# atomicarchitects/equiformer

Measured on NVIDIA H100. Metric: edges/sec fwd+bwd, QM9 Lmax=2 batch, higher is better.
Workload: dtype f32

## Files before the change

### equiformer_b200/csrc/eqf_gemm_tf32x3.cu

```cuda
#include <cuda.h>
#include <cuda_runtime.h>

#include <cstdint>
#include <cstdlib>
#include <mutex>
#include <string>

#include "eqf_common.cuh"
#include "eqf_tc.cuh"

namespace eqf {
namespace tf32x3 {

using namespace tc;

constexpr int BM = 128;
constexpr int BK = kKTile;
constexpr int kRowBytes = BK * 4;
constexpr int kThreads = 384;
constexpr int kConsumerWarps = 8, kConsumerThreads = kConsumerWarps * 32;
constexpr int kSmemBudget = 227 * 1024;
constexpr int kMaxStages = 8;

template <int BN>
// ... 48 lines not shown
    if (++kt == k_tiles) { kt = 0; tile += gridDim.x; }
    const bool more = tile < n_tiles;
    if (more) {
      mbar_wait_hint(&full[s], ph);
      load_a_split(smem_u32(smem + s * S::kStageBytes), row_wg, lane, hn, ln);
    }
    wgmma_wait<0>();
    __syncwarp();
    if (lane == 0) mbar_arrive(&empty[s_cur]);
#pragma unroll
    for (int i = 0; i < BN / 2; ++i) acc[i] = kt_cur == 0 ? part[i] : acc[i] + part[i];
    if (kt_cur == k_tiles - 1) {
      if (leader) bulk_wait_read();
      named_barrier(wg, 128);
      stage_acc<BN>(acc, out, row_w, lane);
      fence_async_smem();
      named_barrier(wg, 128);
      if (leader) {
        const int m0 = (int)(tile_cur / n_blocks) * BM + (wg - 1) * 64;
        const int n0 = (int)(tile_cur % n_blocks) * BN;
#pragma unroll
        for (int b = 0; b < BN / 32; ++b) tma_store_2d(map_c, n0 + 32 * b, m0, out + (uint32_t)b * 8192u);
        bulk_commit();
      }
    }
    return more;
  }
};

template <int BN>
__global__ void __launch_bounds__(kThreads, 1)
gemm_tf32x3_kernel(const __grid_constant__ CUtensorMap map_a, const __grid_constant__ CUtensorMap map_bhi,
                   const __grid_constant__ CUtensorMap map_blo, const __grid_constant__ CUtensorMap map_c, Params p) {
  using S = Smem<BN>;
  constexpr int kStages = S::kStages;
  extern __shared__ uint8_t smem_raw[];
  uint8_t* smem = reinterpret_cast<uint8_t*>((reinterpret_cast<uintptr_t>(smem_raw) + 1023) & ~uintptr_t(1023));
  uint8_t* out_base = smem + kStages * S::kStageBytes;
  uint64_t* full = reinterpret_cast<uint64_t*>(out_base + 2 * S::kOutBytes);
  uint64_t* empty = full + kStages;

  const int warp = threadIdx.x >> 5, lane = threadIdx.x & 31, wg = warp >> 2;
  const int k_tiles = (p.K + BK - 1) / BK;
  if (threadIdx.x == 0) {
    for (int s = 0; s < kStages; ++s) { mbar_init(&full[s], 1); mbar_init(&empty[s], kConsumerWarps); }
    asm volatile("fence.mbarrier_init.release.cluster;" ::: "memory");
  }
  __syncthreads();

  if (wg == 0) {
    reg_dealloc<40>();
    if (threadIdx.x == 0) {
      prefetch_map(&map_a); prefetch_map(&map_bhi); prefetch_map(&map_blo);
      int s = 0;
      uint32_t ph = 0;
      for (long long tile = blockIdx.x; tile < p.n_tiles; tile += gridDim.x) {
        const int m0 = (int)(tile / p.n_blocks) * BM;
        const int n0 = (int)(tile % p.n_blocks) * BN;
        for (int kt = 0; kt < k_tiles; ++kt) {
          mbar_wait_hint(&empty[s], ph ^ 1);
          uint8_t* st = smem + s * S::kStageBytes;
          mbar_expect_tx(&full[s], (uint32_t)S::kStageBytes);
          tma_load_2d(st, &map_a, kt * BK, m0, &full[s]);
          tma_load_2d(st + S::kABytes, &map_bhi, kt * BK, n0, &full[s]);
          tma_load_2d(st + S::kABytes + S::kBBytes, &map_blo, kt * BK, n0, &full[s]);
          if (++s == kStages) { s = 0; ph ^= 1; }
        }
      }
    }
  } else {
    reg_alloc<232>();
    if ((long long)blockIdx.x >= p.n_tiles) return;
    Consumer<BN> c;
    c.smem = smem; c.full = full; c.empty = empty; c.map_c = &map_c;
    c.out = smem_u32(out_base + (wg - 1) * S::kOutBytes);
    c.tile = blockIdx.x; c.n_tiles = p.n_tiles; c.kt = 0; c.k_tiles = k_tiles; c.n_blocks = p.n_blocks;
    c.s = 0; c.ph = 0; c.lane = lane; c.wg = wg;
    c.row_w = (warp & 3) * 16;
    c.row_wg = (wg - 1) * 64 + c.row_w;
    c.leader = (threadIdx.x & 127) == 0;
    if (c.leader) prefetch_map(&map_c);
    uint32_t h0[16], l0[16], h1[16], l1[16];
    mbar_wait_hint(&full[0], 0);
    load_a_split(smem_u32(smem), c.row_wg, lane, h0, l0);
    while (c.step(h0, l0, h1, l1) && c.step(h1, l1, h0, l0)) {}
    if (c.leader) bulk_wait();
  }
}

__global__ void split_kernel(const float* __restrict__ w, float* __restrict__ hi, float* __restrict__ lo, long long n) {
  for (long long i = (long long)blockIdx.x * blockDim.x + threadIdx.x; i < n; i += (long long)gridDim.x * blockDim.x) {
    const float v = w[i];
    const float h = tf32_rn(v);
    hi[i] = h;
    lo[i] = tf32_rn(v - h);
  }
}

__global__ void split_transpose_kernel(const float* __restrict__ w, long long ldw, float* __restrict__ hi,
                                       float* __restrict__ lo, long long N, long long K) {
  const long long n_el = N * K;
  for (long long i = (long long)blockIdx.x * blockDim.x + threadIdx.x; i < n_el; i += (long long)gridDim.x * blockDim.x) {
    const long long n = i / K, k = i - n * K;
    const float v = w[k * ldw + n];
    const float h = tf32_rn(v);
    hi[i] = h;
    lo[i] = tf32_rn(v - h);
  }
}

template <int BN>
static int launch(const CUtensorMap& ma, const CUtensorMap& mh, const CUtensorMap& ml, const CUtensorMap& mc, const Params& p,
                  long long m_blocks, int n_blocks, cudaStream_t s) {
  static std::once_flag once;
  static cudaError_t attr_err = cudaSuccess;
  std::call_once(once, [] {
    attr_err = cudaFuncSetAttribute(gemm_tf32x3_kernel<BN>, cudaFuncAttributeMaxDynamicSharedMemorySize, Smem<BN>::kTotal);
  });
  if (attr_err != cudaSuccess) return check_cuda(attr_err, "gemm_tf32x3 smem attribute");
  Params q = p;
  q.n_blocks = n_blocks;
  q.n_tiles = m_blocks * n_blocks;
  const long long sms = device_sms();
  const unsigned grid = (unsigned)(q.n_tiles < sms ? q.n_tiles : sms);
  gemm_tf32x3_kernel<BN><<<grid, kThreads, Smem<BN>::kTotal, s>>>(ma, mh, ml, mc, q);
  return check_cuda(cudaGetLastError(), "gemm_tf32x3_kernel launch");
}

namespace wg {

constexpr int BKR = BK;
constexpr int kBoxBytes = BKR * 128;
constexpr int kMaxBN = 128;

struct WParams {
  float* out;
  long long R, rows_per_slice, K1;
  int N;
  int reduce;
};

template <int BN>
struct WSmem {
  static constexpr int kABytes = (BM / 32) * kBoxBytes;
  static constexpr int kGRawBytes = BKR * BN * 4;
  static constexpr int kGBytes = BN * kRowBytes;
  static constexpr int kStageBytes = kABytes + kGRawBytes + 2 * kGBytes;
  static constexpr int kStagesRaw = (kSmemBudget - 2048) / kStageBytes;
  static constexpr int kStages = kStagesRaw > kMaxStages ? kMaxStages : kStagesRaw;
  static_assert(kStages >= 2, "tile does not fit shared memory");
  static constexpr int kTotal = kStages * kStageBytes + 1024 + 1024;
};

__device__ __forceinline__ void load_at_split(uint32_t tile, int row0, int lane, uint32_t (&hi)[16], uint32_t (&lo)[16]) {
  const int g = row0 + (lane >> 2), t = lane & 3;
#pragma unroll
  for (int kb = 0; kb < BKR / 8; ++kb) {
#pragma unroll
    for (int q = 0; q < 4; ++q) {
      const int m = g + ((q & 1) ? 8 : 0);
      const int r = kb * 8 + t + ((q & 2) ? 4 : 0);
      const int c = m & 31;
      const uint32_t addr = tile + (uint32_t)(m >> 5) * kBoxBytes + (uint32_t)r * 128u + (uint32_t)((((c >> 2) ^ (r & 7)) << 4) + (c & 3) * 4);
      const float x = lds32(addr);
      const float h = tf32_rn_fast(x);
      hi[kb * 4 + q] = __float_as_uint(h);
      lo[kb * 4 + q] = __float_as_uint(tf32_rn_fast(x - h));
    }
  }
}

template <int BN>
__global__ void __launch_bounds__(kThreads, 1)
wgrad_tf32x3_kernel(const __grid_constant__ CUtensorMap map_a, const __grid_constant__ CUtensorMap map_g, WParams p) {
  using S = WSmem<BN>;
  constexpr int kStages = S::kStages;
  extern __shared__ uint8_t smem_raw[];
  uint8_t* smem = reinterpret_cast<uint8_t*>((reinterpret_cast<uintptr_t>(smem_raw) + 1023) & ~uintptr_t(1023));
  uint64_t* full = reinterpret_cast<uint64_t*>(smem + kStages * S::kStageBytes);
  uint64_t* empty = full + kStages;

  const int warp = threadIdx.x >> 5, lane = threadIdx.x & 31, wgi = warp >> 2;
  const int m0 = blockIdx.x * BM;
  const int n0 = blockIdx.y * BN;
  const long long r_begin = (long long)blockIdx.z * p.rows_per_slice;
  long long r_end = r_begin + p.rows_per_slice;
  if (r_end > p.R) r_end = p.R;
  const int k_tiles = (int)((r_end - r_begin + BKR - 1) / BKR);
  if (threadIdx.x == 0) {
    for (int s = 0; s < kStages; ++s) { mbar_init(&full[s], 1); mbar_init(&empty[s], kConsumerWarps); }
    asm volatile("fence.mbarrier_init.release.cluster;" ::: "memory");
  }
  __syncthreads();

  if (wgi == 0) {
    reg_dealloc<40>();
    if (threadIdx.x == 0) {
      prefetch_map(&map_a); prefetch_map(&map_g);
      for (int kt = 0; kt < k_tiles; ++kt) {
        const int s = kt % kStages;
        mbar_wait_hint(&empty[s], ((kt / kStages) & 1) ^ 1);
        uint8_t* st = smem + s * S::kStageBytes;
        const int r = (int)(r_begin + (long long)kt * BKR);
        mbar_expect_tx(&full[s], (uint32_t)(S::kABytes + S::kGRawBytes));
#pragma unroll
        for (int b = 0; b < BM / 32; ++b) tma_load_2d(st + b * kBoxBytes, &map_a, m0 + 32 * b, r, &full[s]);
        tma_load_2d(st + S::kABytes, &map_g, n0, r, &full[s]);
      }
    }
  } else {
    reg_alloc<232>();
    const int ct = threadIdx.x - 128;
    const int row_wg = (wgi - 1) * 64 + (warp & 3) * 16;
    auto transpose_split = [&](int s) {
      const uint32_t g_raw = smem_u32(smem + s * S::kStageBytes) + S::kABytes, g_hi = g_raw + S::kGRawBytes,
                     g_lo = g_hi + S::kGBytes;
      for (int i = ct; i < BN * (BKR / 4); i += kConsumerThreads) {
        const int n = i % BN, rq = i / BN;
        float4 v;
        v.x = lds32(g_raw + (uint32_t)((4 * rq + 0) * BN + n) * 4u);
        v.y = lds32(g_raw + (uint32_t)((4 * rq + 1) * BN + n) * 4u);
        v.z = lds32(g_raw + (uint32_t)((4 * rq + 2) * BN + n) * 4u);
        v.w = lds32(g_raw + (uint32_t)((4 * rq + 3) * BN + n) * 4u);
        float4 h;
        h.x = tf32_rn_fast(v.x); h.y = tf32_rn_fast(v.y); h.z = tf32_rn_fast(v.z); h.w = tf32_rn_fast(v.w);
        const uint32_t off = (uint32_t)n * 128u + (uint32_t)((rq ^ (n & 7)) << 4);
        sts128(g_hi + off, h);
        sts128(g_lo + off, make_float4(tf32_rn_fast(v.x - h.x), tf32_rn_fast(v.y - h.y), tf32_rn_fast(v.z - h.z),
                                       tf32_rn_fast(v.w - h.w)));
      }
      fence_async_smem();
    };
    float acc[BN / 2], part[BN / 2];
    int kt = 0;
    auto step = [&](const uint32_t (&hc)[16], const uint32_t (&lc)[16], uint32_t (&hn)[16], uint32_t (&ln)[16]) {
      const int s = kt % kStages;
      const uint32_t g_hi = smem_u32(smem + s * S::kStageBytes) + S::kABytes + S::kGRawBytes;
      mma_ktile_3xtf32<BN, true>(part, hc, lc, g_hi, g_hi + S::kGBytes);
      const bool more = kt + 1 < k_tiles;
      if (more) {
        const int s1 = (kt + 1) % kStages;
        mbar_wait_hint(&full[s1], ((kt + 1) / kStages) & 1);
        transpose_split(s1);
        load_at_split(smem_u32(smem + s1 * S::kStageBytes), row_wg, lane, hn, ln);
      }
      wgmma_wait<0>();
      __syncwarp();
      if (lane == 0) mbar_arrive(&empty[s]);
#pragma unroll
      for (int i = 0; i < BN / 2; ++i) acc[i] = kt == 0 ? part[i] : acc[i] + part[i];
      if (more) named_barrier(1, kConsumerThreads);
      ++kt;
      return more;
    };
    uint32_t h0[16], l0[16], h1[16], l1[16];
    mbar_wait_hint(&full[0], 0);
    transpose_split(0);
    load_at_split(smem_u32(smem), row_wg, lane, h0, l0);
    named_barrier(1, kConsumerThreads);
    while (step(h0, l0, h1, l1) && step(h1, l1, h0, l0)) {}
    float* out = p.reduce ? p.out : p.out + (long long)blockIdx.z * p.K1 * p.N;
    store_acc<BN>(acc, out, p.N, m0 + row_wg, p.K1, n0, p.N, lane, p.reduce != 0);
  }
}

struct Shape { int n_tile, n_tiles, m_tiles; long long slices, rows_per_slice; };

static Shape plan(long long R, long long K1, long long N) {
  Shape sh;
  sh.n_tiles = (int)((N + kMaxBN - 1) / kMaxBN);
  sh.n_tile = sh.n_tiles == 1 ? (int)((N + 31) & ~31LL) : kMaxBN;
  sh.m_tiles = (int)((K1 + BM - 1) / BM);
  const long long sms = device_sms();
  long long slices = sms / ((long long)sh.m_tiles * sh.n_tiles);
  if (slices < 1) slices = 1;
  long long rps = (R + slices - 1) / slices;
  if (rps < 64) rps = 64;
  rps = (rps + BKR - 1) / BKR * BKR;
  sh.rows_per_slice = rps;
  sh.slices = (R + rps - 1) / rps;
  return sh;
}

template <int BN>
static int launch(const CUtensorMap& ma, const CUtensorMap& mg, const WParams& p, const Shape& sh, cudaStream_t s) {
  static std::once_flag once;
  static cudaError_t attr_err = cudaSuccess;
  std::call_once(once, [] {
    attr_err = cudaFuncSetAttribute(wgrad_tf32x3_kernel<BN>, cudaFuncAttributeMaxDynamicSharedMemorySize, WSmem<BN>::kTotal);
  });
  if (attr_err != cudaSuccess) return check_cuda(attr_err, "wgrad_tf32x3 smem attribute");
  dim3 grid((unsigned)sh.m_tiles, (unsigned)sh.n_tiles, (unsigned)sh.slices);
  wgrad_tf32x3_kernel<BN><<<grid, kThreads, WSmem<BN>::kTotal, s>>>(ma, mg, p);
  return check_cuda(cudaGetLastError(), "wgrad_tf32x3_kernel launch");
}

}
}
}

using namespace eqf;

extern "C" int eqf_gemm_tf32x3(const float* A, const float* Bt, float* C, int64_t M, int64_t N, int64_t K, int64_t lda,
                               int64_t ldb, int64_t ldc, int32_t b_is_kn, float* split, void* stream) {
  using namespace eqf::tf32x3;
  if (M <= 0 || N <= 0) return EQF_OK;
  if (!A || !Bt || !C || !split) { set_error("eqf_gemm_tf32x3: null pointer"); return EQF_ERR_INVALID; }
  if (K <= 0) { set_error("eqf_gemm_tf32x3: K must be positive"); return EQF_ERR_INVALID; }
  if ((((uintptr_t)A | (uintptr_t)C | (uintptr_t)split) & 15) || ((K | lda | ldc) & 3) || lda < K || ldc < N ||
      ldb < (b_is_kn ? N : K)) {
    set_error("eqf_gemm_tf32x3: operands must be 16-byte aligned, K and leading dimensions multiples of 4");
    return EQF_ERR_INVALID;
  }
  if (K > 0x7fffffffLL || N > 0x7fffffffLL) { set_error("eqf_gemm_tf32x3: K / N too large"); return EQF_ERR_UNSUPPORTED; }
  cudaStream_t s = (cudaStream_t)stream;
  float* hi = split;
  float* lo = split + N * K;
  {
    const long long n = N * K;
    const unsigned blocks = (unsigned)((n + 255) / 256 < 1056 ? (n + 255) / 256 : 1056);
    if (b_is_kn) split_transpose_kernel<<<blocks, 256, 0, s>>>(Bt, ldb, hi, lo, N, K);
    else if (ldb == K) split_kernel<<<blocks, 256, 0, s>>>(Bt, hi, lo, n);
    else { set_error("eqf_gemm_tf32x3: Bt must be packed (ldb == K)"); return EQF_ERR_UNSUPPORTED; }
  }
  int rc = check_cuda(cudaGetLastError(), "split_kernel launch");
  if (rc != EQF_OK) return rc;
  const long long n_split = (N + 127) / 128;
  const long long per = (N + n_split - 1) / n_split;
  const int bn = per <= 32 ? 32 : per <= 64 ? 64 : per <= 96 ? 96 : 128;
  const int n_blocks = (int)((N + bn - 1) / bn);
  const long long m_blocks = (M + BM - 1) / BM;
  if (M > 0x7fffffffLL) { set_error("eqf_gemm_tf32x3: M too large"); return EQF_ERR_UNSUPPORTED; }
  Params p;
  p.N = (int)N; p.K = (int)K;
  CUtensorMap ma, mh, ml, mc;
  if ((rc = make_map_2d(&ma, A, M, K, lda, BM, BK)) != EQF_OK) return rc;
  if ((rc = make_map_2d(&mh, hi, N, K, K, bn, BK)) != EQF_OK) return rc;
  if ((rc = make_map_2d(&ml, lo, N, K, K, bn, BK)) != EQF_OK) return rc;
  if ((rc = make_map_2d(&mc, C, M, N, ldc, 64, 32)) != EQF_OK) return rc;
  switch (bn) {
    case 32: return launch<32>(ma, mh, ml, mc, p, m_blocks, n_blocks, s);
    case 64: return launch<64>(ma, mh, ml, mc, p, m_blocks, n_blocks, s);
    case 96: return launch<96>(ma, mh, ml, mc, p, m_blocks, n_blocks, s);
    default: return launch<128>(ma, mh, ml, mc, p, m_blocks, n_blocks, s);
  }
}

extern "C" int64_t eqf_gemm_tf32x3_wgrad_slices(int64_t R, int64_t K1, int64_t N) {
  if (R <= 0 || K1 <= 0 || N <= 0) return 0;
  return eqf::tf32x3::wg::plan(R, K1, N).slices;
}

static int wgrad_impl(const float* A, const float* G, float* out, bool reduce, int64_t R, int64_t K1, int64_t N,
                      int64_t lda, int64_t ldg, void* stream, const char* who) {
  using namespace eqf::tf32x3;
  if (R <= 0 || K1 <= 0 || N <= 0) return EQF_OK;
  if (!A || !G || !out) { set_error(std::string(who) + ": null pointer"); return EQF_ERR_INVALID; }
  if ((((uintptr_t)A | (uintptr_t)G | (uintptr_t)out) & 15) || ((K1 | N | lda | ldg) & 3) || lda < K1 || ldg < N) {
    set_error(std::string(who) + ": operands must be 16-byte aligned, dimensions multiples of 4");
    return EQF_ERR_INVALID;
  }
  if (R > 0x7fffffffLL || K1 > 0x7fffffffLL || N > 0x7fffffffLL) {
    set_error(std::string(who) + ": too many rows");
    return EQF_ERR_UNSUPPORTED;
  }
  const wg::Shape sh = wg::plan(R, K1, N);
  wg::WParams p;
  p.out = out; p.R = R; p.rows_per_slice = sh.rows_per_slice; p.K1 = K1; p.N = (int)N; p.reduce = reduce ? 1 : 0;
  CUtensorMap ma, mg;
  int rc;
  if ((rc = make_map_2d(&ma, A, R, K1, lda, wg::BKR, 32)) != EQF_OK) return rc;
  if ((rc = make_map_2d(&mg, G, R, N, ldg, wg::BKR, sh.n_tile, MapKind::kLinear)) != EQF_OK) return rc;
  cudaStream_t s = (cudaStream_t)stream;
  if (reduce && (rc = check_cuda(cudaMemsetAsync(out, 0, (size_t)K1 * N * sizeof(float), s), "wgrad memset")) != EQF_OK)
    return rc;
  if (sh.n_tile <= 32) return wg::launch<32>(ma, mg, p, sh, s);
  if (sh.n_tile <= 64) return wg::launch<64>(ma, mg, p, sh, s);
  if (sh.n_tile <= 96) return wg::launch<96>(ma, mg, p, sh, s);
  return wg::launch<128>(ma, mg, p, sh, s);
}

extern "C" int eqf_gemm_tf32x3_wgrad(const float* A, const float* G, float* partial, int64_t R, int64_t K1, int64_t N,
                                     int64_t lda, int64_t ldg, void* stream) {
  return wgrad_impl(A, G, partial, false, R, K1, N, lda, ldg, stream, "eqf_gemm_tf32x3_wgrad");
}

extern "C" int eqf_gemm_tf32x3_wgrad_accumulate(const float* A, const float* G, float* W, int64_t R, int64_t K1, int64_t N,
                                                int64_t lda, int64_t ldg, void* stream) {
  return wgrad_impl(A, G, W, true, R, K1, N, lda, ldg, stream, "eqf_gemm_tf32x3_wgrad_accumulate");
}
```

### equiformer_b200/csrc/eqf_tc.cuh

```cuda
#pragma once
#include <cuda.h>
#include <cuda_runtime.h>

#include <cstdint>
#include <string>

#include "eqf_common.cuh"

namespace eqf {
namespace tc {

__device__ __forceinline__ uint32_t smem_u32(const void* p) { return (uint32_t)__cvta_generic_to_shared(p); }

__device__ __forceinline__ void mbar_init(uint64_t* bar, uint32_t count) {
  asm volatile("mbarrier.init.shared::cta.b64 [%0], %1;" ::"r"(smem_u32(bar)), "r"(count));
}
__device__ __forceinline__ void mbar_arrive(uint64_t* bar) {
  asm volatile("mbarrier.arrive.shared::cta.b64 _, [%0];" ::"r"(smem_u32(bar)) : "memory");
}
__device__ __forceinline__ void mbar_expect_tx(uint64_t* bar, uint32_t bytes) {
  asm volatile("mbarrier.arrive.expect_tx.shared::cta.b64 _, [%0], %1;" ::"r"(smem_u32(bar)), "r"(bytes) : "memory");
}
__device__ __forceinline__ void mbar_wait_hint(uint64_t* bar, uint32_t parity) {
  asm volatile(
      "{\n\t.reg .pred p;\n\t"
      "WAIT_%=:\n\t"
      "mbarrier.try_wait.parity.shared::cta.b64 p, [%0], %1, %2;\n\t"
      "@p bra DONE_%=;\n\t"
      "bra WAIT_%=;\n\t"
      "DONE_%=:\n\t}"
      ::"r"(smem_u32(bar)), "r"(parity), "r"(0x989680u) : "memory");
}
__device__ __forceinline__ void tma_load_2d(void* dst, const CUtensorMap* map, int c0, int c1, uint64_t* bar) {
  asm volatile("cp.async.bulk.tensor.2d.shared::cluster.global.mbarrier::complete_tx::bytes [%0], [%1, {%2, %3}], [%4];"
               ::"r"(smem_u32(dst)), "l"(reinterpret_cast<uint64_t>(map)), "r"(c0), "r"(c1), "r"(smem_u32(bar)) : "memory");
}
__device__ __forceinline__ void tma_store_2d(const CUtensorMap* map, int c0, int c1, uint32_t src) {
  asm volatile("cp.async.bulk.tensor.2d.global.shared::cta.bulk_group [%0, {%1, %2}], [%3];"
               ::"l"(reinterpret_cast<uint64_t>(map)), "r"(c0), "r"(c1), "r"(src) : "memory");
}
__device__ __forceinline__ void bulk_commit() { asm volatile("cp.async.bulk.commit_group;" ::: "memory"); }
__device__ __forceinline__ void bulk_wait_read() { asm volatile("cp.async.bulk.wait_group.read 0;" ::: "memory"); }
__device__ __forceinline__ void bulk_wait() { asm volatile("cp.async.bulk.wait_group 0;" ::: "memory"); }
__device__ __forceinline__ void prefetch_map(const CUtensorMap* map) {
  asm volatile("prefetch.tensormap [%0];" ::"l"(reinterpret_cast<uint64_t>(map)) : "memory");
}
__device__ __forceinline__ void fence_async_smem() { asm volatile("fence.proxy.async.shared::cta;" ::: "memory"); }

__device__ __forceinline__ float tf32_rn(float x) {
  uint32_t r;
  asm("cvt.rna.tf32.f32 %0, %1;" : "=r"(r) : "f"(x));
  return __uint_as_float(r);
}
__device__ __forceinline__ float tf32_rn_fast(float x) {
  return __uint_as_float((__float_as_uint(x) + 0x1000u) & 0xffffe000u);
}

__device__ __forceinline__ float lds32(uint32_t addr) {
  float v;
  asm volatile("ld.shared.f32 %0, [%1];" : "=f"(v) : "r"(addr));
  return v;
}
__device__ __forceinline__ float4 lds128(uint32_t addr) {
  float4 v;
  asm volatile("ld.shared.v4.f32 {%0, %1, %2, %3}, [%4];" : "=f"(v.x), "=f"(v.y), "=f"(v.z), "=f"(v.w) : "r"(addr));
  return v;
}
__device__ __forceinline__ void sts128(uint32_t addr, const float4& v) {
  asm volatile("st.shared.v4.f32 [%0], {%1, %2, %3, %4};" ::"r"(addr), "f"(v.x), "f"(v.y), "f"(v.z), "f"(v.w) : "memory");
}

template <int N> __device__ __forceinline__ void reg_alloc() { asm volatile("setmaxnreg.inc.sync.aligned.u32 %0;" ::"n"(N)); }
template <int N> __device__ __forceinline__ void reg_dealloc() { asm volatile("setmaxnreg.dec.sync.aligned.u32 %0;" ::"n"(N)); }

__device__ __forceinline__ void named_barrier(int id, int threads) {
  asm volatile("bar.sync %0, %1;" ::"r"(id), "r"(threads) : "memory");
}

__device__ __forceinline__ uint64_t smem_desc_sw128(uint32_t addr) {
  return (uint64_t)((addr >> 4) & 0x3FFF) | (1ull << 16) | (64ull << 32) | (1ull << 62);
}
__device__ __forceinline__ void wgmma_fence() { asm volatile("wgmma.fence.sync.aligned;" ::: "memory"); }
__device__ __forceinline__ void wgmma_commit() { asm volatile("wgmma.commit_group.sync.aligned;" ::: "memory"); }
template <int N> __device__ __forceinline__ void wgmma_wait() { asm volatile("wgmma.wait_group.sync.aligned %0;" ::"n"(N) : "memory"); }

template <int kScaleD = 1>
__device__ __forceinline__ void wgmma_rs_n32(float* d, const uint32_t* a, uint64_t b_desc) {
  asm volatile(
      "{\n\t.reg .pred p;\n\tsetp.ne.b32 p, %21, 0;\n\t"
      "wgmma.mma_async.sync.aligned.m64n32k8.f32.tf32.tf32 "
      "{%0, %1, %2, %3, %4, %5, %6, %7, %8, %9, %10, %11, %12, %13, %14, %15}, "
      "{%16, %17, %18, %19}, %20, p, 1, 1;\n\t}"
      : "+f"(d[0]), "+f"(d[1]), "+f"(d[2]), "+f"(d[3]), "+f"(d[4]), "+f"(d[5]), "+f"(d[6]), "+f"(d[7]),
        "+f"(d[8]), "+f"(d[9]), "+f"(d[10]), "+f"(d[11]), "+f"(d[12]), "+f"(d[13]), "+f"(d[14]), "+f"(d[15])
      : "r"(a[0]), "r"(a[1]), "r"(a[2]), "r"(a[3]), "l"(b_desc), "n"(kScaleD));
}
template <int kScaleD = 1>
__device__ __forceinline__ void wgmma_rs_n64(float* d, const uint32_t* a, uint64_t b_desc) {
  asm volatile(
      "{\n\t.reg .pred p;\n\tsetp.ne.b32 p, %37, 0;\n\t"
      "wgmma.mma_async.sync.aligned.m64n64k8.f32.tf32.tf32 "
      "{%0, %1, %2, %3, %4, %5, %6, %7, %8, %9, %10, %11, %12, %13, %14, %15, "
      "%16, %17, %18, %19, %20, %21, %22, %23, %24, %25, %26, %27, %28, %29, %30, %31}, "
      "{%32, %33, %34, %35}, %36, p, 1, 1;\n\t}"
      : "+f"(d[0]), "+f"(d[1]), "+f"(d[2]), "+f"(d[3]), "+f"(d[4]), "+f"(d[5]), "+f"(d[6]), "+f"(d[7]),
        "+f"(d[8]), "+f"(d[9]), "+f"(d[10]), "+f"(d[11]), "+f"(d[12]), "+f"(d[13]), "+f"(d[14]), "+f"(d[15]),
        "+f"(d[16]), "+f"(d[17]), "+f"(d[18]), "+f"(d[19]), "+f"(d[20]), "+f"(d[21]), "+f"(d[22]), "+f"(d[23]),
        "+f"(d[24]), "+f"(d[25]), "+f"(d[26]), "+f"(d[27]), "+f"(d[28]), "+f"(d[29]), "+f"(d[30]), "+f"(d[31])
      : "r"(a[0]), "r"(a[1]), "r"(a[2]), "r"(a[3]), "l"(b_desc), "n"(kScaleD));
}

template <int kScaleD = 1>
__device__ __forceinline__ void wgmma_rs_n96(float* d, const uint32_t* a, uint64_t b_desc) {
  asm volatile(
      "{\n\t.reg .pred p;\n\tsetp.ne.b32 p, %53, 0;\n\t"
      "wgmma.mma_async.sync.aligned.m64n96k8.f32.tf32.tf32 "
      "{%0, %1, %2, %3, %4, %5, %6, %7, %8, %9, %10, %11, %12, %13, %14, %15, "
      "%16, %17, %18, %19, %20, %21, %22, %23, %24, %25, %26, %27, %28, %29, %30, %31, "
      "%32, %33, %34, %35, %36, %37, %38, %39, %40, %41, %42, %43, %44, %45, %46, %47}, "
      "{%48, %49, %50, %51}, %52, p, 1, 1;\n\t}"
      : "+f"(d[0]), "+f"(d[1]), "+f"(d[2]), "+f"(d[3]), "+f"(d[4]), "+f"(d[5]), "+f"(d[6]), "+f"(d[7]),
        "+f"(d[8]), "+f"(d[9]), "+f"(d[10]), "+f"(d[11]), "+f"(d[12]), "+f"(d[13]), "+f"(d[14]), "+f"(d[15]),
        "+f"(d[16]), "+f"(d[17]), "+f"(d[18]), "+f"(d[19]), "+f"(d[20]), "+f"(d[21]), "+f"(d[22]), "+f"(d[23]),
        "+f"(d[24]), "+f"(d[25]), "+f"(d[26]), "+f"(d[27]), "+f"(d[28]), "+f"(d[29]), "+f"(d[30]), "+f"(d[31]),
        "+f"(d[32]), "+f"(d[33]), "+f"(d[34]), "+f"(d[35]), "+f"(d[36]), "+f"(d[37]), "+f"(d[38]), "+f"(d[39]),
        "+f"(d[40]), "+f"(d[41]), "+f"(d[42]), "+f"(d[43]), "+f"(d[44]), "+f"(d[45]), "+f"(d[46]), "+f"(d[47])
// ... 37 lines not shown
      const float h = tf32_rn_fast(x);
      hi[kb * 4 + q] = __float_as_uint(h);
      lo[kb * 4 + q] = __float_as_uint(tf32_rn_fast(x - h));
    }
  }
}

template <int BN, bool kFresh = false, int N4>
__device__ __forceinline__ void mma_ktile_3xtf32(float* acc, const uint32_t (&hi)[N4], const uint32_t (&lo)[N4], uint32_t b_hi,
                                                 uint32_t b_lo, int kb0 = 0) {
  static_assert(BN % 32 == 0 && BN >= 32 && BN <= 256, "BN must be a multiple of 32 up to 256");
  wgmma_fence();
#pragma unroll
  for (int kb = 0; kb < N4 / 4; ++kb) {
    const uint64_t adv = (uint64_t)(((kb0 + kb) * 32) >> 4);
    if constexpr (BN == 96 || BN == 128) {
      const uint64_t dh = smem_desc_sw128(b_hi) + adv, dl = smem_desc_sw128(b_lo) + adv;
      if constexpr (BN == 96) {
        if (kFresh && kb == 0) wgmma_rs_n96<0>(acc, &lo[kb * 4], dh);
        else wgmma_rs_n96(acc, &lo[kb * 4], dh);
        wgmma_rs_n96(acc, &hi[kb * 4], dl);
        wgmma_rs_n96(acc, &hi[kb * 4], dh);
      } else {
        if (kFresh && kb == 0) wgmma_rs_n128<0>(acc, &lo[kb * 4], dh);
        else wgmma_rs_n128(acc, &lo[kb * 4], dh);
        wgmma_rs_n128(acc, &hi[kb * 4], dl);
        wgmma_rs_n128(acc, &hi[kb * 4], dh);
      }
    } else {
#pragma unroll
      for (int j = 0; j < BN / 64; ++j) {
        const uint64_t dh = smem_desc_sw128(b_hi + (uint32_t)j * 8192u) + adv, dl = smem_desc_sw128(b_lo + (uint32_t)j * 8192u) + adv;
        if (kFresh && kb == 0) wgmma_rs_n64<0>(acc + 32 * j, &lo[kb * 4], dh);
        else wgmma_rs_n64(acc + 32 * j, &lo[kb * 4], dh);
        wgmma_rs_n64(acc + 32 * j, &hi[kb * 4], dl);
        wgmma_rs_n64(acc + 32 * j, &hi[kb * 4], dh);
      }
      if constexpr (BN % 64 == 32) {
        constexpr int j = BN / 64;
        const uint64_t dh = smem_desc_sw128(b_hi + (uint32_t)j * 8192u) + adv, dl = smem_desc_sw128(b_lo + (uint32_t)j * 8192u) + adv;
        if (kFresh && kb == 0) wgmma_rs_n32<0>(acc + 32 * j, &lo[kb * 4], dh);
        else wgmma_rs_n32(acc + 32 * j, &lo[kb * 4], dh);
        wgmma_rs_n32(acc + 32 * j, &hi[kb * 4], dl);
        wgmma_rs_n32(acc + 32 * j, &hi[kb * 4], dh);
      }
    }
  }
  wgmma_commit();
}

__device__ __forceinline__ int acc_row(int i, int lane) { return (lane >> 2) + ((i >> 1) & 1) * 8; }
__device__ __forceinline__ int acc_col(int i, int lane) { return 8 * ((i & 31) >> 2) + 2 * (lane & 3) + (i & 1) + 64 * (i >> 5); }

template <int BN>
__device__ __forceinline__ void store_acc(const float* acc, float* C, long long ldc, long long row0, long long M, int col0, int N,
                                          int lane, bool add) {
#pragma unroll
  for (int i = 0; i < BN / 2; i += 2) {
    const long long r = row0 + acc_row(i, lane);
    const int c = col0 + acc_col(i, lane);
    if (r >= M || c >= N) continue;
    float* p = C + r * ldc + c;
    if (add) {
      atomicAdd(p, acc[i]);
      if (c + 1 < N) atomicAdd(p + 1, acc[i + 1]);
    } else if (c + 1 < N) {
      *reinterpret_cast<float2*>(p) = make_float2(acc[i], acc[i + 1]);
    } else {
      *p = acc[i];
    }
  }
}

typedef CUresult (*EncodeTiled)(CUtensorMap*, CUtensorMapDataType, cuuint32_t, void*, const cuuint64_t*, const cuuint64_t*,
                                const cuuint32_t*, const cuuint32_t*, CUtensorMapInterleave, CUtensorMapSwizzle,
                                CUtensorMapL2promotion, CUtensorMapFloatOOBfill);

static inline EncodeTiled encode_fn() {
  static EncodeTiled fn = [] {
    void* f = nullptr;
    cudaDriverEntryPointQueryResult q;
    if (cudaGetDriverEntryPoint("cuTensorMapEncodeTiled", &f, cudaEnableDefault, &q) != cudaSuccess) f = nullptr;
    return reinterpret_cast<EncodeTiled>(f);
  }();
  return fn;
}

enum class MapKind { kSwizzled, kLinear };

static inline int make_map_2d(CUtensorMap* map, const float* base, long long rows, long long cols, long long ld, int box_rows,
                              int box_cols, MapKind kind = MapKind::kSwizzled) {
  EncodeTiled enc = encode_fn();
  if (enc == nullptr) { set_error("cuTensorMapEncodeTiled is not available from the driver"); return EQF_ERR_CUDA; }
  cuuint64_t dims[2] = {(cuuint64_t)cols, (cuuint64_t)rows};
  cuuint64_t strides[1] = {(cuuint64_t)ld * sizeof(float)};
  cuuint32_t box[2] = {(cuuint32_t)box_cols, (cuuint32_t)box_rows};
  cuuint32_t estr[2] = {1, 1};
  const CUtensorMapSwizzle sw = kind == MapKind::kLinear ? CU_TENSOR_MAP_SWIZZLE_NONE : CU_TENSOR_MAP_SWIZZLE_128B;
  CUresult r = enc(map, CU_TENSOR_MAP_DATA_TYPE_FLOAT32, 2, const_cast<float*>(base), dims, strides, box, estr,
                   CU_TENSOR_MAP_INTERLEAVE_NONE, sw, CU_TENSOR_MAP_L2_PROMOTION_L2_128B, CU_TENSOR_MAP_FLOAT_OOB_FILL_NONE);
  if (r != CUDA_SUCCESS) { set_error("cuTensorMapEncodeTiled failed (code " + std::to_string((int)r) + ")"); return EQF_ERR_CUDA; }
  return EQF_OK;
}

static inline int device_sms() {
  int sms = 132, dev = 0;
  cudaGetDevice(&dev);
  cudaDeviceGetAttribute(&sms, cudaDevAttrMultiProcessorCount, dev);
  return sms;
}

}
}
```

### equiformer_b200/csrc/eqf_fused.cu

```cuda
#include <cuda.h>
#include <cuda_runtime.h>

#include <cstdint>
#include <mutex>
#include <string>
#include <vector>

#include "eqf_common.cuh"
#include "eqf_tc.cuh"

namespace eqf {
namespace fused {

using namespace tc;

constexpr int BM = 128;
constexpr int BKT = kKTile;
constexpr int kRowBytes = BKT * 4;
constexpr int kProducerWarp = 4;
constexpr int kHelperWarp0 = 6, kHelperWarps = 2, kHelperThreads = kHelperWarps * 32;
constexpr int kConsumerWarps = 8;
constexpr int kDtpWarp0 = 12, kDtpWarps = 16, kDtpSets = 2, kDtpSetWarps = kDtpWarps / kDtpSets;
constexpr int kDtpSetThreads = kDtpSetWarps * 32;
constexpr int kThreads = (kDtpWarp0 + kDtpWarps) * 32;
// ... 186 lines not shown
  const long long n_tiles_total = a.m_blocks * a.n_blocks;
  const bool w_tma = !a.w_shared;

  if (threadIdx.x == kProducerWarp * 32) {
    prefetch_map(&map_bhi); prefetch_map(&map_blo);
    if (w_tma) prefetch_map(&map_w);
    for (int s = 0; s < kMaxStages; ++s) {
      mbar_init(&op_full[s], 1);
      mbar_init(&op_empty[s], kConsumerWarps);
      mbar_init(&raw_ready[s], kDtpSetWarps);
      mbar_init(&raw_free[s], kConsumerWarps);
    }
    for (int b = 0; b < 2; ++b) {
      mbar_init(&tab_ready[b], kHelperWarps);
      mbar_init(&tab_free[b], kDtpWarps);
    }
    asm volatile("fence.mbarrier_init.release.cluster;" ::: "memory");
  }
  __syncthreads();

  if (warp < 4 || (warp >= 8 && warp < kDtpWarp0)) {
    reg_alloc<80>();
    const int row_wg = (warp < 4 ? 0 : 64) + (warp & 3) * 16;
    const bool stamper = threadIdx.x == 0;
    Ring op(n_op), raw(n_raw);
    int n_stamp = 0;
    for (long long tile = blockIdx.x; tile < n_tiles_total; tile += gridDim.x) {
      const long long mb = tile / a.n_blocks;
      const int nb = (int)(tile % a.n_blocks);
      float acc[BN / 2];
#pragma unroll
      for (int i = 0; i < BN / 2; ++i) acc[i] = 0.f;
      for (int kt = 0; kt < k_tiles; ++kt, op.next(), raw.next()) {
        mbar_wait_hint(&op_full[op.idx], op.ph);
        mbar_wait_hint(&raw_ready[raw.idx], raw.ph);
        if (stamper) stamp(a, 1, n_stamp);
        const uint32_t raw_tile = smem_u32(raw_base + (size_t)raw.idx * S::kABytes);
        const uint32_t st = smem_u32(op_base + (size_t)op.idx * a.op_bytes);
#pragma unroll
        for (int half = 0; half < 2; ++half) {
          uint32_t hi[8], lo[8];
          load_a_split(raw_tile, row_wg, lane, hi, lo, 2 * half);
          if (half == 1) {
            __syncwarp();
            if (lane == 0) mbar_arrive(&raw_free[raw.idx]);
          }
          mma_ktile_3xtf32<BN>(acc, hi, lo, st, st + S::kBBytes, 2 * half);
          wgmma_wait<0>();
        }
        __syncwarp();
        if (lane == 0) mbar_arrive(&op_empty[op.idx]);
        if (stamper) stamp(a, 1, n_stamp);
      }
      store_acc<BN>(acc, a.C, a.ldc, mb * BM + row_wg, a.M, nb * BN, a.N, lane, false);
      if (stamper) stamp(a, 3, n_stamp);
    }
  } else if (warp < 8) {
    reg_dealloc<56>();
    if (warp == kProducerWarp) {
      if (lane == 0) {
        Ring op(n_op);
        int n_stamp = 0;
        const uint32_t tx = (uint32_t)(2 * S::kBBytes) + (w_tma ? (uint32_t)(a.w_box_rows * kRowBytes) : 0u);
        for (long long tile = blockIdx.x; tile < n_tiles_total; tile += gridDim.x) {
          const long long mb = tile / a.n_blocks;
          const int nb = (int)(tile % a.n_blocks);
          const int e0 = (int)((mb * BM) / d3);
          for (int kt = 0; kt < k_tiles; ++kt, op.next()) {
            mbar_wait_hint(&op_empty[op.idx], op.ph ^ 1);
            stamp(a, 0, n_stamp);
            uint8_t* st = op_base + (size_t)op.idx * a.op_bytes;
            mbar_expect_tx(&op_full[op.idx], tx);
            tma_load_2d(st, &map_bhi, kt * BKT, nb * BN, &op_full[op.idx]);
            tma_load_2d(st + S::kBBytes, &map_blo, kt * BKT, nb * BN, &op_full[op.idx]);
            if (w_tma) {
              const FPath& p = a.paths[a.kt_path[kt]];
              tma_load_2d(st + a.w_tile_off, &map_w, p.w_off + (kt * BKT - p.koff), e0, &op_full[op.idx]);
            }
          }
        }
      }
    } else if (warp >= kHelperWarp0) {
      const int ht = threadIdx.x - kHelperWarp0 * 32;
      const int m_row = a.m_row, d_y = a.d_y;
      {
        int off = 0;
        for (int pi = 0; pi < a.n_paths; ++pi) {
          const FPath& p = a.paths[pi];
          const int n = p.d1 * p.d2 * d3;
          for (int i = ht; i < n; i += kHelperThreads) cg_s[off + i] = __ldg(a.cg + p.cg_off + i);
          off += n;
        }
        for (int q = ht; q < m_row; q += kHelperThreads) {
          int pi = 0, cg0 = 0;
          for (int j = 1; j < a.n_paths; ++j) if (q >= a.paths[j].m_off) pi = j;
          for (int j = 0; j < pi; ++j) cg0 += a.paths[j].d1 * a.paths[j].d2 * d3;
          const FPath& p = a.paths[pi];
          const int r = q - p.m_off;
          const int i = r / d3, k = r - i * d3;
          if (i < p.d1) mdesc[q] = make_int4(cg0 + i * p.d2 * d3 + k, p.y_off, p.d2, 0);
          else mdesc[q] = make_int4(0, 0, 0, 0);
        }
        named_barrier(2, kHelperThreads);
      }
      const uint32_t cg_addr = smem_u32(cg_s);
      uint32_t tile_it = 0;
      int n_stamp = 0;
// ... 376 lines not shown
```

Baseline: 1.436 million.

## Use programmatic dependent launch for tf32x3 GEMMs and vectorize wgrad atomics

Launches the forward GEMM and the reducing wgrad kernel with programmatic stream serialization. The preceding split/zero kernels trigger dependents early, and the consumer kernels call griddepcontrol.wait before their dependent reads or stores, so prologue and mainloop work can overlap the previous kernel's tail. The memset becomes a PDL-triggering zero kernel, and paired scalar atomicAdds become float2 atomicAdd. The risk is ordering: in the forward GEMM only the producer waits, and correctness assumes the consumer never reads memory written by the predecessor except through the producer's loads.

```diff
diff --git a/equiformer_b200/csrc/eqf_gemm_tf32x3.cu b/equiformer_b200/csrc/eqf_gemm_tf32x3.cu
--- a/equiformer_b200/csrc/eqf_gemm_tf32x3.cu
+++ b/equiformer_b200/csrc/eqf_gemm_tf32x3.cu
@@ -124,6 +124,7 @@
     reg_dealloc<40>();
     if (threadIdx.x == 0) {
       prefetch_map(&map_a); prefetch_map(&map_bhi); prefetch_map(&map_blo);
+      pdl_wait();
       int s = 0;
       uint32_t ph = 0;
       for (long long tile = blockIdx.x; tile < p.n_tiles; tile += gridDim.x) {
@@ -160,7 +161,30 @@
   }
 }
 
+template <typename... KArgs, typename... Args>
+static cudaError_t launch_dependent(void (*kernel)(KArgs...), dim3 grid, int smem, cudaStream_t s, bool dependent,
+                                    const Args&... args) {
+  cudaLaunchConfig_t cfg = {};
+  cfg.gridDim = grid;
+  cfg.blockDim = dim3(kThreads);
+  cfg.dynamicSmemBytes = (size_t)smem;
+  cfg.stream = s;
+  cudaLaunchAttribute attr[1];
+  attr[0].id = cudaLaunchAttributeProgrammaticStreamSerialization;
+  attr[0].val.programmaticStreamSerializationAllowed = 1;
+  cfg.attrs = attr;
+  cfg.numAttrs = dependent ? 1 : 0;
+  return cudaLaunchKernelEx(&cfg, kernel, args...);
+}
+
+__global__ void zero_kernel(float4* __restrict__ w, long long n4) {
+  pdl_trigger();
+  for (long long i = (long long)blockIdx.x * blockDim.x + threadIdx.x; i < n4; i += (long long)gridDim.x * blockDim.x)
+    w[i] = make_float4(0.f, 0.f, 0.f, 0.f);
+}
+
 __global__ void split_kernel(const float* __restrict__ w, float* __restrict__ hi, float* __restrict__ lo, long long n) {
+  pdl_trigger();
   for (long long i = (long long)blockIdx.x * blockDim.x + threadIdx.x; i < n; i += (long long)gridDim.x * blockDim.x) {
     const float v = w[i];
     const float h = tf32_rn(v);
@@ -171,6 +195,7 @@
 
 __global__ void split_transpose_kernel(const float* __restrict__ w, long long ldw, float* __restrict__ hi,
                                        float* __restrict__ lo, long long N, long long K) {
+  pdl_trigger();
   const long long n_el = N * K;
   for (long long i = (long long)blockIdx.x * blockDim.x + threadIdx.x; i < n_el; i += (long long)gridDim.x * blockDim.x) {
     const long long n = i / K, k = i - n * K;
@@ -195,8 +220,8 @@
   q.n_tiles = m_blocks * n_blocks;
   const long long sms = device_sms();
   const unsigned grid = (unsigned)(q.n_tiles < sms ? q.n_tiles : sms);
-  gemm_tf32x3_kernel<BN><<<grid, kThreads, Smem<BN>::kTotal, s>>>(ma, mh, ml, mc, q);
-  return check_cuda(cudaGetLastError(), "gemm_tf32x3_kernel launch");
+  return check_cuda(launch_dependent(gemm_tf32x3_kernel<BN>, dim3(grid), Smem<BN>::kTotal, s, true, ma, mh, ml, mc, q),
+                    "gemm_tf32x3_kernel launch");
 }
 
 namespace wg {
@@ -332,6 +357,7 @@
     named_barrier(1, kConsumerThreads);
     while (step(h0, l0, h1, l1) && step(h1, l1, h0, l0)) {}
     float* out = p.reduce ? p.out : p.out + (long long)blockIdx.z * p.K1 * p.N;
+    pdl_wait();
     store_acc<BN>(acc, out, p.N, m0 + row_wg, p.K1, n0, p.N, lane, p.reduce != 0);
   }
 }
@@ -363,8 +389,8 @@
   });
   if (attr_err != cudaSuccess) return check_cuda(attr_err, "wgrad_tf32x3 smem attribute");
   dim3 grid((unsigned)sh.m_tiles, (unsigned)sh.n_tiles, (unsigned)sh.slices);
-  wgrad_tf32x3_kernel<BN><<<grid, kThreads, WSmem<BN>::kTotal, s>>>(ma, mg, p);
-  return check_cuda(cudaGetLastError(), "wgrad_tf32x3_kernel launch");
+  return check_cuda(launch_dependent(wgrad_tf32x3_kernel<BN>, grid, WSmem<BN>::kTotal, s, p.reduce != 0, ma, mg, p),
+                    "wgrad_tf32x3_kernel launch");
 }
 
 }
@@ -444,8 +470,11 @@
   if ((rc = make_map_2d(&ma, A, R, K1, lda, wg::BKR, 32)) != EQF_OK) return rc;
   if ((rc = make_map_2d(&mg, G, R, N, ldg, wg::BKR, sh.n_tile, MapKind::kLinear)) != EQF_OK) return rc;
   cudaStream_t s = (cudaStream_t)stream;
-  if (reduce && (rc = check_cuda(cudaMemsetAsync(out, 0, (size_t)K1 * N * sizeof(float), s), "wgrad memset")) != EQF_OK)
-    return rc;
+  if (reduce) {
+    const long long n4 = K1 * N / 4;
+    zero_kernel<<<(unsigned)((n4 + 255) / 256 < 264 ? (n4 + 255) / 256 : 264), 256, 0, s>>>(reinterpret_cast<float4*>(out), n4);
+    if ((rc = check_cuda(cudaGetLastError(), "zero_kernel launch")) != EQF_OK) return rc;
+  }
   if (sh.n_tile <= 32) return wg::launch<32>(ma, mg, p, sh, s);
   if (sh.n_tile <= 64) return wg::launch<64>(ma, mg, p, sh, s);
   if (sh.n_tile <= 96) return wg::launch<96>(ma, mg, p, sh, s);
diff --git a/equiformer_b200/csrc/eqf_tc.cuh b/equiformer_b200/csrc/eqf_tc.cuh
--- a/equiformer_b200/csrc/eqf_tc.cuh
+++ b/equiformer_b200/csrc/eqf_tc.cuh
@@ -72,6 +72,9 @@
 
 template <int N> __device__ __forceinline__ void reg_alloc() { asm volatile("setmaxnreg.inc.sync.aligned.u32 %0;" ::"n"(N)); }
 template <int N> __device__ __forceinline__ void reg_dealloc() { asm volatile("setmaxnreg.dec.sync.aligned.u32 %0;" ::"n"(N)); }
+
+__device__ __forceinline__ void pdl_trigger() { asm volatile("griddepcontrol.launch_dependents;" ::: "memory"); }
+__device__ __forceinline__ void pdl_wait() { asm volatile("griddepcontrol.wait;" ::: "memory"); }
 
 __device__ __forceinline__ void named_barrier(int id, int threads) {
   asm volatile("bar.sync %0, %1;" ::"r"(id), "r"(threads) : "memory");
@@ -225,8 +228,8 @@
     if (r >= M || c >= N) continue;
     float* p = C + r * ldc + c;
     if (add) {
-      atomicAdd(p, acc[i]);
-      if (c + 1 < N) atomicAdd(p + 1, acc[i + 1]);
+      if (c + 1 < N) atomicAdd(reinterpret_cast<float2*>(p), make_float2(acc[i], acc[i + 1]));
+      else atomicAdd(p, acc[i]);
     } else if (c + 1 < N) {
       *reinterpret_cast<float2*>(p) = make_float2(acc[i], acc[i + 1]);
     } else {
```

Result: no change. 1.428 million, median of 6 (-0.6%).

## Batch multiple K-tiles per stage in narrow wgrad and vectorize loads and reductions

Applied to the files above, without the earlier changes.

For narrow weight-gradient tiles (BN at most 32), each pipeline stage now carries four K-tiles of rows, so the mbarrier waits, named barriers and transposes are amortised over more work. The A-fragment loader uses paired-row 64-bit shared loads, with matching permutations in the G transpose and the output store. The reduce path switches from scalar atomicAdd to shuffle-assembled red.global.add.v4.f32. The trade is larger stages, hence fewer of them, and more complex indexing that must stay exactly consistent with the permuted row order.

```diff
diff --git a/equiformer_b200/csrc/eqf_fused.cu b/equiformer_b200/csrc/eqf_fused.cu
--- a/equiformer_b200/csrc/eqf_fused.cu
+++ b/equiformer_b200/csrc/eqf_fused.cu
@@ -262,7 +262,7 @@
         if (lane == 0) mbar_arrive(&op_empty[op.idx]);
         if (stamper) stamp(a, 1, n_stamp);
       }
-      store_acc<BN>(acc, a.C, a.ldc, mb * BM + row_wg, a.M, nb * BN, a.N, lane, false);
+      store_acc<BN>(acc, a.C, a.ldc, mb * BM + row_wg, a.M, nb * BN, a.N, lane);
       if (stamper) stamp(a, 3, n_stamp);
     }
   } else if (warp < 8) {
diff --git a/equiformer_b200/csrc/eqf_gemm_tf32x3.cu b/equiformer_b200/csrc/eqf_gemm_tf32x3.cu
--- a/equiformer_b200/csrc/eqf_gemm_tf32x3.cu
+++ b/equiformer_b200/csrc/eqf_gemm_tf32x3.cu
@@ -201,8 +201,7 @@
 
 namespace wg {
 
-constexpr int BKR = BK;
-constexpr int kBoxBytes = BKR * 128;
+template <int BN> constexpr int kSub = BN <= 32 ? 4 : 1;
 constexpr int kMaxBN = 128;
 
 struct WParams {
@@ -214,31 +213,50 @@
 
 template <int BN>
 struct WSmem {
+  static constexpr int kRows = kSub<BN> * BK;
+  static constexpr int kBoxBytes = kRows * 128;
   static constexpr int kABytes = (BM / 32) * kBoxBytes;
-  static constexpr int kGRawBytes = BKR * BN * 4;
+  static constexpr int kGRawBytes = kRows * BN * 4;
   static constexpr int kGBytes = BN * kRowBytes;
-  static constexpr int kStageBytes = kABytes + kGRawBytes + 2 * kGBytes;
+  static constexpr int kStageBytes = kABytes + kGRawBytes + 2 * kSub<BN> * kGBytes;
   static constexpr int kStagesRaw = (kSmemBudget - 2048) / kStageBytes;
   static constexpr int kStages = kStagesRaw > kMaxStages ? kMaxStages : kStagesRaw;
   static_assert(kStages >= 2, "tile does not fit shared memory");
   static constexpr int kTotal = kStages * kStageBytes + 1024 + 1024;
 };
 
+template <int kBoxBytes>
 __device__ __forceinline__ void load_at_split(uint32_t tile, int row0, int lane, uint32_t (&hi)[16], uint32_t (&lo)[16]) {
-  const int g = row0 + (lane >> 2), t = lane & 3;
-#pragma unroll
-  for (int kb = 0; kb < BKR / 8; ++kb) {
-#pragma unroll
-    for (int q = 0; q < 4; ++q) {
-      const int m = g + ((q & 1) ? 8 : 0);
-      const int r = kb * 8 + t + ((q & 2) ? 4 : 0);
-      const int c = m & 31;
-      const uint32_t addr = tile + (uint32_t)(m >> 5) * kBoxBytes + (uint32_t)r * 128u + (uint32_t)((((c >> 2) ^ (r & 7)) << 4) + (c & 3) * 4);
-      const float x = lds32(addr);
-      const float h = tf32_rn_fast(x);
-      hi[kb * 4 + q] = __float_as_uint(h);
-      lo[kb * 4 + q] = __float_as_uint(tf32_rn_fast(x - h));
+  const int m = row0 + 2 * (lane >> 2), t = lane & 3, c = m & 31;
+  const uint32_t base = tile + (uint32_t)(m >> 5) * kBoxBytes + (uint32_t)(c & 3) * 4;
+#pragma unroll
+  for (int kb = 0; kb < BK / 8; ++kb) {
+#pragma unroll
+    for (int h = 0; h < 2; ++h) {
+      const int r = kb * 8 + 2 * t + h;
+      const float2 x = lds64(base + (uint32_t)r * 128u + (uint32_t)(((c >> 2) ^ (r & 7)) << 4));
+      const float h0 = tf32_rn_fast(x.x), h1 = tf32_rn_fast(x.y);
+      hi[kb * 4 + 2 * h] = __float_as_uint(h0);
+      hi[kb * 4 + 2 * h + 1] = __float_as_uint(h1);
+      lo[kb * 4 + 2 * h] = __float_as_uint(tf32_rn_fast(x.x - h0));
+      lo[kb * 4 + 2 * h + 1] = __float_as_uint(tf32_rn_fast(x.y - h1));
     }
+  }
+}
+
+template <int BN>
+__device__ __forceinline__ void add_acc(const float* acc, float* W, int N, long long row0, long long K1, int col0, int lane) {
+  const bool odd = lane & 1;
+  const long long r = row0 + 2 * (lane >> 2) + (odd ? 1 : 0);
+#pragma unroll
+  for (int i = 0; i < BN / 2; i += 4) {
+    const float s0 = __shfl_xor_sync(0xffffffffu, odd ? acc[i] : acc[i + 2], 1);
+    const float s1 = __shfl_xor_sync(0xffffffffu, odd ? acc[i + 1] : acc[i + 3], 1);
+    const int c = col0 + acc_col(i, lane & ~1);
+    if (r >= K1 || c >= N) continue;
+    const float4 v = odd ? make_float4(s0, s1, acc[i + 2], acc[i + 3]) : make_float4(acc[i], acc[i + 1], s0, s1);
+    asm volatile("red.global.add.v4.f32 [%0], {%1, %2, %3, %4};" ::"l"(W + r * N + c), "f"(v.x), "f"(v.y), "f"(v.z), "f"(v.w)
+                 : "memory");
   }
 }
 
@@ -246,7 +264,7 @@
 __global__ void __launch_bounds__(kThreads, 1)
 wgrad_tf32x3_kernel(const __grid_constant__ CUtensorMap map_a, const __grid_constant__ CUtensorMap map_g, WParams p) {
   using S = WSmem<BN>;
-  constexpr int kStages = S::kStages;
+  constexpr int kStages = S::kStages, KS = kSub<BN>;
   extern __shared__ uint8_t smem_raw[];
   uint8_t* smem = reinterpret_cast<uint8_t*>((reinterpret_cast<uintptr_t>(smem_raw) + 1023) & ~uintptr_t(1023));
   uint64_t* full = reinterpret_cast<uint64_t*>(smem + kStages * S::kStageBytes);
@@ -258,7 +276,8 @@
   const long long r_begin = (long long)blockIdx.z * p.rows_per_slice;
   long long r_end = r_begin + p.rows_per_slice;
   if (r_end > p.R) r_end = p.R;
-  const int k_tiles = (int)((r_end - r_begin + BKR - 1) / BKR);
+  const int k_tiles = (int)((r_end - r_begin + BK - 1) / BK);
+  const int n_stages = (k_tiles + KS - 1) / KS;
   if (threadIdx.x == 0) {
     for (int s = 0; s < kStages; ++s) { mbar_init(&full[s], 1); mbar_init(&empty[s], kConsumerWarps); }
     asm volatile("fence.mbarrier_init.release.cluster;" ::: "memory");
@@ -269,86 +288,98 @@
     reg_dealloc<40>();
     if (threadIdx.x == 0) {
       prefetch_map(&map_a); prefetch_map(&map_g);
-      for (int kt = 0; kt < k_tiles; ++kt) {
-        const int s = kt % kStages;
-        mbar_wait_hint(&empty[s], ((kt / kStages) & 1) ^ 1);
-        uint8_t* st = smem + s * S::kStageBytes;
-        const int r = (int)(r_begin + (long long)kt * BKR);
+      for (int st = 0; st < n_stages; ++st) {
+        const int s = st % kStages;
+        mbar_wait_hint(&empty[s], ((st / kStages) & 1) ^ 1);
+        uint8_t* sp = smem + s * S::kStageBytes;
+        const int r = (int)(r_begin + (long long)st * S::kRows);
         mbar_expect_tx(&full[s], (uint32_t)(S::kABytes + S::kGRawBytes));
 #pragma unroll
-        for (int b = 0; b < BM / 32; ++b) tma_load_2d(st + b * kBoxBytes, &map_a, m0 + 32 * b, r, &full[s]);
-        tma_load_2d(st + S::kABytes, &map_g, n0, r, &full[s]);
+        for (int b = 0; b < BM / 32; ++b) tma_load_2d(sp + b * S::kBoxBytes, &map_a, m0 + 32 * b, r, &full[s]);
+        tma_load_2d(sp + S::kABytes, &map_g, n0, r, &full[s]);
       }
     }
   } else {
     reg_alloc<232>();
     const int ct = threadIdx.x - 128;
     const int row_wg = (wgi - 1) * 64 + (warp & 3) * 16;
+    auto g_hi = [&](int s, int j) { return smem_u32(smem + s * S::kStageBytes) + S::kABytes + S::kGRawBytes + j * S::kGBytes; };
     auto transpose_split = [&](int s) {
-      const uint32_t g_raw = smem_u32(smem + s * S::kStageBytes) + S::kABytes, g_hi = g_raw + S::kGRawBytes,
-                     g_lo = g_hi + S::kGBytes;
-      for (int i = ct; i < BN * (BKR / 4); i += kConsumerThreads) {
+      const uint32_t g_raw = smem_u32(smem + s * S::kStageBytes) + S::kABytes;
+      for (int i = ct; i < BN * (S::kRows / 4); i += kConsumerThreads) {
         const int n = i % BN, rq = i / BN;
+        const int r0 = (rq >> 3) * BK + ((rq & 7) >> 1) * 8 + (rq & 1);
         float4 v;
-        v.x = lds32(g_raw + (uint32_t)((4 * rq + 0) * BN + n) * 4u);
-        v.y = lds32(g_raw + (uint32_t)((4 * rq + 1) * BN + n) * 4u);
-        v.z = lds32(g_raw + (uint32_t)((4 * rq + 2) * BN + n) * 4u);
-        v.w = lds32(g_raw + (uint32_t)((4 * rq + 3) * BN + n) * 4u);
+        v.x = lds32(g_raw + (uint32_t)((r0 + 0) * BN + n) * 4u);
+        v.y = lds32(g_raw + (uint32_t)((r0 + 2) * BN + n) * 4u);
+        v.z = lds32(g_raw + (uint32_t)((r0 + 4) * BN + n) * 4u);
+        v.w = lds32(g_raw + (uint32_t)((r0 + 6) * BN + n) * 4u);
         float4 h;
         h.x = tf32_rn_fast(v.x); h.y = tf32_rn_fast(v.y); h.z = tf32_rn_fast(v.z); h.w = tf32_rn_fast(v.w);
-        const uint32_t off = (uint32_t)n * 128u + (uint32_t)((rq ^ (n & 7)) << 4);
-        sts128(g_hi + off, h);
-        sts128(g_lo + off, make_float4(tf32_rn_fast(v.x - h.x), tf32_rn_fast(v.y - h.y), tf32_rn_fast(v.z - h.z),
-                                       tf32_rn_fast(v.w - h.w)));
+        const uint32_t hi = g_hi(s, rq >> 3), off = (uint32_t)n * 128u + (uint32_t)(((rq & 7) ^ (n & 7)) << 4);
+        sts128(hi + off, h);
+        sts128(hi + KS * S::kGBytes + off, make_float4(tf32_rn_fast(v.x - h.x), tf32_rn_fast(v.y - h.y),
+                                                       tf32_rn_fast(v.z - h.z), tf32_rn_fast(v.w - h.w)));
       }
       fence_async_smem();
+    };
+    auto load_split = [&](int kt, uint32_t (&h)[16], uint32_t (&l)[16]) {
+      const uint32_t a = smem_u32(smem + ((kt / KS) % kStages) * S::kStageBytes) + (uint32_t)(kt % KS) * (BK * 128u);
+      load_at_split<S::kBoxBytes>(a, row_wg, lane, h, l);
     };
     float acc[BN / 2], part[BN / 2];
     int kt = 0;
     auto step = [&](const uint32_t (&hc)[16], const uint32_t (&lc)[16], uint32_t (&hn)[16], uint32_t (&ln)[16]) {
-      const int s = kt % kStages;
-      const uint32_t g_hi = smem_u32(smem + s * S::kStageBytes) + S::kABytes + S::kGRawBytes;
-      mma_ktile_3xtf32<BN, true>(part, hc, lc, g_hi, g_hi + S::kGBytes);
+      const int st = kt / KS, s = st % kStages;
+      const uint32_t ghi = g_hi(s, kt % KS);
+      mma_ktile_3xtf32<BN, true>(part, hc, lc, ghi, ghi + KS * S::kGBytes);
       const bool more = kt + 1 < k_tiles;
+      const bool opens = more && (kt + 1) % KS == 0;
       if (more) {
-        const int s1 = (kt + 1) % kStages;
-        mbar_wait_hint(&full[s1], ((kt + 1) / kStages) & 1);
-        transpose_split(s1);
-        load_at_split(smem_u32(smem + s1 * S::kStageBytes), row_wg, lane, hn, ln);
+        if (opens) {
+          const int st1 = st + 1;
+          mbar_wait_hint(&full[st1 % kStages], (st1 / kStages) & 1);
+          transpose_split(st1 % kStages);
+        }
+        load_split(kt + 1, hn, ln);
       }
       wgmma_wait<0>();
-      __syncwarp();
-      if (lane == 0) mbar_arrive(&empty[s]);
+      if (opens) {
+        __syncwarp();
+        if (lane == 0) mbar_arrive(&empty[s]);
+      }
 #pragma unroll
       for (int i = 0; i < BN / 2; ++i) acc[i] = kt == 0 ? part[i] : acc[i] + part[i];
-      if (more) named_barrier(1, kConsumerThreads);
+      if (opens) named_barrier(1, kConsumerThreads);
       ++kt;
       return more;
     };
     uint32_t h0[16], l0[16], h1[16], l1[16];
     mbar_wait_hint(&full[0], 0);
     transpose_split(0);
-    load_at_split(smem_u32(smem), row_wg, lane, h0, l0);
+    load_split(0, h0, l0);
     named_barrier(1, kConsumerThreads);
     while (step(h0, l0, h1, l1) && step(h1, l1, h0, l0)) {}
-    float* out = p.reduce ? p.out : p.out + (long long)blockIdx.z * p.K1 * p.N;
-    store_acc<BN>(acc, out, p.N, m0 + row_wg, p.K1, n0, p.N, lane, p.reduce != 0);
-  }
-}
-
-struct Shape { int n_tile, n_tiles, m_tiles; long long slices, rows_per_slice; };
+    if (p.reduce) add_acc<BN>(acc, p.out, p.N, m0 + row_wg, p.K1, n0, lane);
+    else store_acc<BN, true>(acc, p.out + (long long)blockIdx.z * p.K1 * p.N, p.N, m0 + row_wg, p.K1, n0, p.N, lane);
+  }
+}
+
+struct Shape { int n_tile, n_tiles, m_tiles, stage_rows; long long slices, rows_per_slice; };
 
 static Shape plan(long long R, long long K1, long long N) {
   Shape sh;
   sh.n_tiles = (int)((N + kMaxBN - 1) / kMaxBN);
   sh.n_tile = sh.n_tiles == 1 ? (int)((N + 31) & ~31LL) : kMaxBN;
+  sh.stage_rows = sh.n_tile <= 32 ? WSmem<32>::kRows : sh.n_tile <= 64 ? WSmem<64>::kRows : sh.n_tile <= 96 ? WSmem<96>::kRows
+                                                                                          : WSmem<128>::kRows;
   sh.m_tiles = (int)((K1 + BM - 1) / BM);
   const long long sms = device_sms();
   long long slices = sms / ((long long)sh.m_tiles * sh.n_tiles);
   if (slices < 1) slices = 1;
   long long rps = (R + slices - 1) / slices;
   if (rps < 64) rps = 64;
-  rps = (rps + BKR - 1) / BKR * BKR;
+  rps = (rps + sh.stage_rows - 1) / sh.stage_rows * sh.stage_rows;
   sh.rows_per_slice = rps;
   sh.slices = (R + rps - 1) / rps;
   return sh;
@@ -441,8 +472,8 @@
   p.out = out; p.R = R; p.rows_per_slice = sh.rows_per_slice; p.K1 = K1; p.N = (int)N; p.reduce = reduce ? 1 : 0;
   CUtensorMap ma, mg;
   int rc;
-  if ((rc = make_map_2d(&ma, A, R, K1, lda, wg::BKR, 32)) != EQF_OK) return rc;
-  if ((rc = make_map_2d(&mg, G, R, N, ldg, wg::BKR, sh.n_tile, MapKind::kLinear)) != EQF_OK) return rc;
+  if ((rc = make_map_2d(&ma, A, R, K1, lda, sh.stage_rows, 32)) != EQF_OK) return rc;
+  if ((rc = make_map_2d(&mg, G, R, N, ldg, sh.stage_rows, sh.n_tile, MapKind::kLinear)) != EQF_OK) return rc;
   cudaStream_t s = (cudaStream_t)stream;
   if (reduce && (rc = check_cuda(cudaMemsetAsync(out, 0, (size_t)K1 * N * sizeof(float), s), "wgrad memset")) != EQF_OK)
     return rc;
diff --git a/equiformer_b200/csrc/eqf_tc.cuh b/equiformer_b200/csrc/eqf_tc.cuh
--- a/equiformer_b200/csrc/eqf_tc.cuh
+++ b/equiformer_b200/csrc/eqf_tc.cuh
@@ -59,6 +59,11 @@
 __device__ __forceinline__ float lds32(uint32_t addr) {
   float v;
   asm volatile("ld.shared.f32 %0, [%1];" : "=f"(v) : "r"(addr));
+  return v;
+}
+__device__ __forceinline__ float2 lds64(uint32_t addr) {
+  float2 v;
+  asm volatile("ld.shared.v2.f32 {%0, %1}, [%2];" : "=f"(v.x), "=f"(v.y) : "r"(addr));
   return v;
 }
 __device__ __forceinline__ float4 lds128(uint32_t addr) {
@@ -215,19 +220,16 @@
 __device__ __forceinline__ int acc_row(int i, int lane) { return (lane >> 2) + ((i >> 1) & 1) * 8; }
 __device__ __forceinline__ int acc_col(int i, int lane) { return 8 * ((i & 31) >> 2) + 2 * (lane & 3) + (i & 1) + 64 * (i >> 5); }
 
-template <int BN>
+template <int BN, bool kPairedRows = false>
 __device__ __forceinline__ void store_acc(const float* acc, float* C, long long ldc, long long row0, long long M, int col0, int N,
-                                          int lane, bool add) {
+                                          int lane) {
 #pragma unroll
   for (int i = 0; i < BN / 2; i += 2) {
-    const long long r = row0 + acc_row(i, lane);
+    const long long r = row0 + (kPairedRows ? 2 * (lane >> 2) + ((i >> 1) & 1) : acc_row(i, lane));
     const int c = col0 + acc_col(i, lane);
     if (r >= M || c >= N) continue;
     float* p = C + r * ldc + c;
-    if (add) {
-      atomicAdd(p, acc[i]);
-      if (c + 1 < N) atomicAdd(p + 1, acc[i + 1]);
-    } else if (c + 1 < N) {
+    if (c + 1 < N) {
       *reinterpret_cast<float2*>(p) = make_float2(acc[i], acc[i + 1]);
     } else {
       *p = acc[i];
```

New measurement: 1.431 million before, 1.471 million after, median of 6. +2.8%, better.
